# debbiemarkslab/BEAR

Measured on AMD Instinct MI355X. Metric: k-mer contexts/sec (DM-marginal+grad h), k=13, higher is better.
Workload: dtype f64

## Files before the change

### bear_amd/csrc/kernels_plan.h

```cpp
#pragma once
#include "plan_common.h"

__global__ __launch_bounds__(256) void plan_scan_kernel(const uint32_t *__restrict__ counts, uint64_t n_rows, int ncol,
                                                        uint8_t *__restrict__ quad_light,
                                                        unsigned long long *__restrict__ heavy_counts,
                                                        unsigned long long *__restrict__ hist) {
  __shared__ uint32_t s_heavy[3];
  __shared__ uint32_t s_hist[2 * SRT_NKEY];
  __shared__ uint32_t s_big[PLN_NBIG + 1];
  __shared__ unsigned long long s_total, s_cells;
  __shared__ uint32_t s_cmax;
  unsigned long long my_total = 0ull;
  uint32_t my_cells = 0u, my_cmax = 0u;
  if (threadIdx.x == 0) {
    s_total = s_cells = 0ull;
    s_cmax = 0u;
  }
  if (threadIdx.x < 3) s_heavy[threadIdx.x] = 0;
  if (threadIdx.x < 2 * SRT_NKEY) s_hist[threadIdx.x] = 0;
  for (uint32_t k = threadIdx.x; k <= PLN_NBIG; k += 256) s_big[k] = 0;
  __syncthreads();
  const uint64_t n_quads = (n_rows + PLN_QUAD - 1) / PLN_QUAD;
  for (uint64_t g = (uint64_t)blockIdx.x * 256 + threadIdx.x; g < n_quads; g += (uint64_t)gridDim.x * 256) {
    uint32_t light = 0, qhc = 0, qhr = 0;
// ... 154 lines not shown
    }
    meta[1] = run;
    meta[2] = run > 0xffffffffull ? 1ull : 0ull;
  }
  __syncthreads();
  unsigned long long off = part[threadIdx.x];
  for (uint64_t t = lo; t < hi; ++t) {
    tiles[t].off16 = (uint32_t)off;
    off += tiles[t].blk16;
  }
}

__global__ __launch_bounds__(1024) void plan_fill_kernel(const uint32_t *__restrict__ counts, uint64_t n_rows, int ncol,
                                                         const pln_tile *__restrict__ tiles, uint64_t n_tiles,
                                                         unsigned char *__restrict__ stream,
                                                         pln_heavy_col *__restrict__ heavy_col,
                                                         pln_heavy_row *__restrict__ heavy_row,
                                                         uint64_t *__restrict__ heavy_stop,
                                                         unsigned long long *__restrict__ cursors) {
  constexpr int RPT = (PLN_RMAX + 1023) / 1024;
  __shared__ uint32_t hist[SRT_NHIST];
  __shared__ uint32_t offs[SRT_NHIST];
  __shared__ uint32_t scan[16];
  __shared__ uint16_t sorted[PLN_NI + 64];
  __shared__ uint32_t s_hc, s_hr;
#ifdef BEAR_DET_BUILD
  __shared__ uint32_t comp[PLN_NI];
  static_assert((PLN_NI & (PLN_NI - 1)) == 0 && PLN_NI <= 2048, "bitonic sort over the tile's items: PLN_NI / 2 pairs, at most one per thread");
  __shared__ unsigned long long hkey[PLN_HCAP], htmp[PLN_HCAP];
#endif
  const uint32_t tid = threadIdx.x, rep = tid & (SRT_REP - 1);
  for (uint64_t t = blockIdx.x; t < n_tiles; t += gridDim.x) {
    const pln_tile ti = tiles[t];
    const uint32_t rows = ti.rows_items >> 16, n_light = ti.rows_items & 0xffffu;
    const uint32_t hc_cap = ti.hc_hr >> 16, hr_cap = ti.hc_hr & 0xffffu;
    const pln_layout L = pln_block_layout(rows, n_light, hc_cap, hr_cap);
    unsigned char *blk = stream + (size_t)ti.off16 * 16;
    uint16_t *E = reinterpret_cast<uint16_t *>(blk);
    uint8_t *nrow = blk + L.nrow;
    uint16_t *items = reinterpret_cast<uint16_t *>(blk + L.items);
    uint16_t *hoff = reinterpret_cast<uint16_t *>(blk + L.hoff);
    uint32_t *hcnt = reinterpret_cast<uint32_t *>(blk + L.hcnt);
    uint16_t *hrow = reinterpret_cast<uint16_t *>(blk + L.hrow);
    double *hn = reinterpret_cast<double *>(blk + L.hn);
    if (tid < SRT_NHIST) hist[tid] = 0;
    if (tid == 0) {
      s_hc = 0;
      s_hr = 0;
    }
    __syncthreads();
#ifdef BEAR_DET_BUILD
    uint32_t det_hc[RPT], det_hr[RPT];
    {
      uint32_t base_c = 0, base_r = 0;
#pragma unroll
      for (int k = 0; k < RPT; ++k) {
        const uint32_t lr = tid + 1024u * k;
        uint32_t nc = 0, nr = 0;
        if (lr < rows) {
          double n = 0.0;
          for (int b = 0; b < 5; ++b) {
            const uint32_t cv = counts[(ti.row0 + lr) * 5 + b];
            n += (double)cv;
            nc += (b < ncol && cv > SRT_CL) ? 1u : 0u;
          }
          nr = n > (double)SRT_CL ? 1u : 0u;
        }
        const uint32_t packed = nc | (nr << 16);
        const int lane = tid & 63, wave = tid >> 6;
        uint32_t incl = packed;
#pragma unroll
        for (int off = 1; off < 64; off <<= 1) {
          const uint32_t o = (uint32_t)__shfl_up((int)incl, off, 64);
          if (lane >= off) incl += o;
        }
        __syncthreads();
        if (lane == 63) scan[wave] = incl;
        __syncthreads();
        uint32_t before = 0, total = 0;
        for (int w = 0; w < 16; ++w) {
          if (w < wave) before += scan[w];
          total += scan[w];
        }
        const uint32_t excl = before + incl - packed;
        det_hc[k] = base_c + (excl & 0xffffu);
        det_hr[k] = base_r + (excl >> 16);
        base_c += total & 0xffffu;
        base_r += total >> 16;
      }
      __syncthreads();
      if (tid == 0) {
        s_hc = base_c;
        s_hr = base_r;
      }
    }
#endif
    uint32_t c[RPT][5], rank[RPT][5];
#pragma unroll
    for (int k = 0; k < RPT; ++k) {
      const uint32_t lr = tid + 1024u * k;
#pragma unroll
      for (int b = 0; b < 5; ++b) {
        c[k][b] = 0;
        rank[k][b] = 0;
      }
      if (lr < rows) {
        const uint64_t r = ti.row0 + lr;
        double n = 0.0;
#pragma unroll
        for (int b = 0; b < 5; ++b) {
          c[k][b] = counts[r * 5 + b];
          n += (double)c[k][b];
        }
        nrow[lr] = n < 1.0 ? (uint8_t)0 : (n <= (double)SRT_CL ? (uint8_t)n : (uint8_t)255);
        if (n > (double)SRT_CL) {
#ifdef BEAR_DET_BUILD
          const uint32_t k2 = hr_cap ? det_hr[k] : 0xffffffffu;
#else
          const uint32_t k2 = hr_cap ? atomicAdd(&s_hr, 1u) : 0xffffffffu;
#endif
          if (k2 < hr_cap) {
            hrow[k2] = (uint16_t)lr;
            hn[k2] = n;
          } else {
            const unsigned long long q = atomicAdd(&cursors[1], 1ull);
            heavy_row[q].row = r;
            heavy_row[q].n = n;
          }
        }
        if (ncol == 4 && c[k][4] > SRT_CL) heavy_stop[atomicAdd(&cursors[2], 1ull)] = c[k][4];
#pragma unroll
        for (int b = 0; b < 5; ++b) {
          if (b >= ncol) c[k][b] = 0;
          if (c[k][b] > SRT_CL) {
#ifdef BEAR_DET_BUILD
            const uint32_t k2 = hc_cap ? det_hc[k]++ : 0xffffffffu;
#else
            const uint32_t k2 = hc_cap ? atomicAdd(&s_hc, 1u) : 0xffffffffu;
#endif
            if (k2 < hc_cap) {
              hoff[k2] = (uint16_t)(lr * 5 + b);
              hcnt[k2] = c[k][b];
            } else {
              const unsigned long long q = atomicAdd(&cursors[0], 1ull);
              heavy_col[q].off = r * 5 + b;
              heavy_col[q].c = c[k][b];
            }
            c[k][b] = 0;
          }
          if (c[k][b] != 0) rank[k][b] = atomicAdd(&hist[(c[k][b] - 1) * SRT_REP + rep], 1u);
        }
      } else if (lr < ((rows + 15u) & ~15u)) {
        nrow[lr] = 0;
      }
    }
    __syncthreads();
    {
      const uint32_t v = tid < SRT_NHIST ? hist[tid] : 0u;
      const int lane = tid & 63, wave = tid >> 6;
      uint32_t incl = v;
#pragma unroll
      for (int off = 1; off < 64; off <<= 1) {
        uint32_t o = (uint32_t)__shfl_up((int)incl, off, 64);
        if (lane >= off) incl += o;
      }
      if (lane == 63) scan[wave] = incl;
      __syncthreads();
      uint32_t base = 0;
      for (int w = 0; w < wave; ++w) base += scan[w];
      if (tid < SRT_NHIST) offs[tid] = base + incl - v;
    }
    __syncthreads();
    if (tid < 30) E[tid] = (uint16_t)(tid < SRT_CL ? offs[tid * SRT_REP] : n_light);
    if (tid == 30) E[30] = (uint16_t)hc_cap;
    if (tid == 31) E[31] = (uint16_t)hr_cap;
#pragma unroll
    for (int k = 0; k < RPT; ++k)
#pragma unroll
      for (int b = 0; b < 5; ++b)
        if (c[k][b] != 0) sorted[offs[(c[k][b] - 1) * SRT_REP + rep] + rank[k][b]] = (uint16_t)((tid + 1024u * k) * 5 + b);
    __syncthreads();
#ifdef BEAR_DET_BUILD
    {
      for (uint32_t i = tid; i < PLN_NI; i += 1024) {
        uint32_t key = 0;
        for (uint32_t q = 1; q < SRT_CL; ++q) key += offs[q * SRT_REP] <= i ? 1u : 0u;
        comp[i] = i < n_light ? (key << 16) | sorted[i] : 0xffffffffu;
      }
      __syncthreads();
      for (uint32_t size = 2; size <= PLN_NI; size <<= 1)
        for (uint32_t stride = size >> 1; stride > 0; stride >>= 1) {
          const uint32_t lo = 2u * tid - (tid & (stride - 1u)), hi = lo + stride;
          if (tid < PLN_NI / 2) {
            const bool up = (lo & size) == 0u;
            const uint32_t a = comp[lo], bq = comp[hi];
            if ((a > bq) == up) {
              comp[lo] = bq;
              comp[hi] = a;
            }
          }
          __syncthreads();
        }
      for (uint32_t i = tid; i < n_light; i += 1024) sorted[i] = (uint16_t)(comp[i] & 0xffffu);
      __syncthreads();
      const uint32_t nhc = s_hc < hc_cap ? s_hc : hc_cap, nhr = s_hr < hr_cap ? s_hr : hr_cap;
      if (tid < nhc) hkey[tid] = ((unsigned long long)hoff[tid] << 32) | hcnt[tid];
      __syncthreads();
      if (tid < nhc) {
        uint32_t r = 0;
        for (uint32_t q = 0; q < nhc; ++q) r += hkey[q] < hkey[tid] ? 1u : 0u;
        htmp[r] = hkey[tid];
      }
      __syncthreads();
      if (tid < nhc) {
        hoff[tid] = (uint16_t)(htmp[tid] >> 32);
        hcnt[tid] = (uint32_t)htmp[tid];
      }
      __syncthreads();
      if (tid < nhr) hkey[tid] = ((unsigned long long)hrow[tid] << 48) | tid;
      if (tid < nhr) htmp[tid] = (unsigned long long)__double_as_longlong(hn[tid]);
      __syncthreads();
      uint32_t r = 0;
      unsigned long long mine = 0ull, myn = 0ull;
      if (tid < nhr) {
        for (uint32_t q = 0; q < nhr; ++q) r += hkey[q] < hkey[tid] ? 1u : 0u;
        mine = hkey[tid];
        myn = htmp[tid];
      }
      __syncthreads();
      if (tid < nhr) {
        hrow[r] = (uint16_t)(mine >> 48);
        hn[r] = __longlong_as_double((long long)myn);
      }
      __syncthreads();
    }
#endif
    const uint32_t padded = (n_light + 63u) & ~63u;
    for (uint32_t i = tid; i < padded; i += 1024) items[i] = i < n_light ? sorted[i] : (uint16_t)PLN_SENTINEL;
    __syncthreads();
  }
}

__global__ __launch_bounds__(1024) void plan_live_kernel(const pln_tile *__restrict__ tiles, uint64_t n_tiles,
                                                         const unsigned char *__restrict__ stream, uint16_t *__restrict__ live) {
  constexpr int RPT = (PLN_RMAX + 1023) / 1024;
  __shared__ uint32_t cnt[RPT * 16];
  const uint32_t tid = threadIdx.x, lane = tid & 63, wave = tid >> 6;
  for (uint64_t t = blockIdx.x; t < n_tiles; t += gridDim.x) {
    const pln_tile ti = tiles[t];
    const uint32_t rows = ti.rows_items >> 16;
    const uint8_t *nrow = stream + (size_t)ti.off16 * 16 + 64;
    uint16_t *out = live + t * PLN_LIVE_STRIDE;
    unsigned long long mask[RPT];
#pragma unroll
    for (int k = 0; k < RPT; ++k) {
      const uint32_t lr = tid + 1024u * k;
      mask[k] = __builtin_amdgcn_ballot_w64(lr < rows && nrow[lr] != 0);
      if (lane == 0) cnt[k * 16 + wave] = (uint32_t)__builtin_popcountll(mask[k]);
    }
    __syncthreads();
    uint32_t total = 0;
#pragma unroll
    for (int k = 0; k < RPT; ++k) {
      uint32_t base = total;
      for (int w = 0; w < 16; ++w) {
        const uint32_t c = cnt[k * 16 + w];
        if (w < (int)wave) base += c;
        total += c;
      }
      if ((mask[k] >> lane) & 1ull) out[1 + base + (uint32_t)__builtin_popcountll(mask[k] & ((1ull << lane) - 1ull))] = (uint16_t)(tid + 1024u * k);
    }
    if (tid == 0) out[0] = (uint16_t)total;
    __syncthreads();
  }
}

template <bool NORM, bool AR>
__global__ __launch_bounds__(PLN_THREADS, 4) void dm_prior_plan_kernel(const double *__restrict__ prior,
                                                                                    uint64_t n_rows, bear_params prm_arg,
                                                                                    pln_view pv,
                                                                                    const double2 *__restrict__ logtab_g,
                                                                                    double *__restrict__ partials,
                                                                                    const bear_step_io io
#ifdef PLN_STAMPS
                                                                                    , unsigned long long *__restrict__ dbg
#endif
                                                                                    ) {
  extern __shared__ __attribute__((aligned(16))) unsigned char srt_smem[];
  pln_lds_n &S = *reinterpret_cast<pln_lds_n *>(srt_smem);
  const bear_params prm = bear_params_of(prm_arg, io);
  const uint32_t tid = threadIdx.x, lane = tid & 63, wave = srt_uniform(tid >> 6);
  const double u = prm.inv_h, eps = prm.eps, eps5 = 5.0 * prm.eps;
  double acc[2] = {0.0, 0.0};

  if (tid < BEAR_LOGTAB_N) S.logtab[tid] = logtab_g[tid];
  if (tid < SRT_NKEY) {
    const bear_dp o = srt_general_fast(u + eps5, (double)(tid + 1), logtab_g);
    S.tabD[tid] = o.D;
    S.tabP[tid] = o.P;
  }
  if (tid < PLN_NBUF) {
    S.buf[tid].pri[PLN_SENTINEL] = 1.0;
    S.ticket[tid] = PLN_TICKET_START(PLN_WAVES - PLN_DMA_WAVES);
    S.sum_fail[tid] = 0xffffffffu;
  }

  const bool dma_wave = wave >= PLN_WAVES - PLN_DMA_WAVES;
  const uint32_t dw = wave - (PLN_WAVES - PLN_DMA_WAVES);
  constexpr bool GEN = !NORM && !AR;
  constexpr bool NT = GEN && PLN_GEN_NT;
  auto stage = [&](const pln_tile &ti, uint32_t b, bool with_nrow) {
    const uint32_t rows = ti.rows_items >> 16;
    if (rows == 0) return;
    const uint32_t pbytes = (rows * 40u) & ~15u, bbytes = ti.blk16 * 16u;
    const unsigned char *psrc = reinterpret_cast<const unsigned char *>(prior + ti.row0 * 5);
    const unsigned char *bsrc = pv.stream + (size_t)ti.off16 * 16;
    if (GEN && dw == 0 && lane == 0) S.nrow_in[b] = with_nrow ? 1u : 0u;
    if (!GEN || with_nrow) {
      for (uint32_t pc = dw; (pc << 10) < bbytes; pc += PLN_DMA_WAVES) pln_dma_piece<NT>(S.buf[b].blk, bsrc, bbytes, pc, lane);
    } else {
      const uint32_t items0 = pln_block_layout(rows, ti.rows_items & 0xffffu, ti.hc_hr >> 16, ti.hc_hr & 0xffffu).items;
      if (dw == PLN_DMA_WAVES - 1) pln_dma_piece<NT>(S.buf[b].blk, bsrc, 64u, 0u, lane);
      for (uint32_t pc = dw; (pc << 10) < bbytes - items0; pc += PLN_DMA_WAVES)
        pln_dma_piece<NT>(S.buf[b].blk + items0, bsrc + items0, bbytes - items0, pc, lane);
    }
    for (uint32_t pc = dw; (pc << 10) < pbytes; pc += PLN_DMA_WAVES) pln_dma_piece<NT>(S.buf[b].pri, psrc, pbytes, pc, lane);
    if (dw == 0 && ((rows * 40u) & 15u)) {
      const __attribute__((address_space(4))) double *tail =
          (const __attribute__((address_space(4))) double *)(uintptr_t)(prior + (ti.row0 + rows) * 5 - 1);
      const double v = *tail;
      if (lane == 0) S.buf[b].pri[rows * 5 - 1] = v;
    }
  };

  constexpr uint32_t PF_INSTR = (NORM || AR || PLN_GEN_PREFETCH) ? PLN_PREFETCH_KIB / 8u : 0u;
  auto prefetch_behind = [&](const pln_tile &ti) -> uint32_t {
    const uint32_t rows = ti.rows_items >> 16;
    if (PF_INSTR == 0 || rows == 0) return 0u;
    const uint64_t end_bytes = n_rows * 40ull, base = (ti.row0 + rows) * 40ull;
    const uint32_t m = srt_uniform((uint32_t)(uintptr_t)S.pf_scratch);
    uint32_t issued = 0;
    for (uint32_t k = dw; k < PF_INSTR; k += PLN_DMA_WAVES) {
      uint64_t off = base + ((uint64_t)(k * 64u + lane) << 7);
      if (off + 4u > end_bytes) off = end_bytes - 4u;
      const unsigned char *g = reinterpret_cast<const unsigned char *>(prior) + off;
      uint32_t keep_m0;
      asm volatile("s_mov_b32 %0, m0\n\ts_mov_b32 m0, %2\n\ts_nop 0\n\tglobal_load_lds_dword %1, off\n\ts_mov_b32 m0, %0"
                   : "=&s"(keep_m0)
                   : "v"(g), "s"(m)
                   : "memory");
      ++issued;
    }
    return issued;
  };
  uint32_t pf_young = 0;
#ifdef PLN_STAMPS
  unsigned long long tph[8] = {0, 0, 0, 0, 0, 0, 0, 0}, t_prev = __builtin_amdgcn_s_memtime();
  int prev_kind = 0;
#define PLN_STAMP(k)                                              \
  {                                                               \
    const unsigned long long now = __builtin_amdgcn_s_memtime();  \
    tph[k] += now - t_prev;                                       \
    t_prev = now;                                                 \
  }
#else
#define PLN_STAMP(k)
#endif
  static_assert(PLN_NBUF == 2, "the DMA-wave protocol below is written for a two-slot ring");
  const uint64_t G = gridDim.x;
  const uint64_t first = (pv.n_tiles * (uint64_t)blockIdx.x) / G, count = (pv.n_tiles * ((uint64_t)blockIdx.x + 1)) / G - first;
  auto fetch_desc = [&](uint64_t j0) {
    if (dw == 0 && j0 < count)
      pln_dma_piece(S.desc[(j0 >> 5) & 1u], pv.tiles + first + j0, PLN_DESC_CHUNK * (uint32_t)sizeof(pln_tile), 0u, lane);
  };
  if (dma_wave) {
    __builtin_amdgcn_s_setprio(3);
    fetch_desc(0);
    fetch_desc(PLN_DESC_CHUNK);
    srt_wait_dma();
  }
  __syncthreads();
  pln_tile cur = pln_desc(S.desc, 0, count), nxt = pln_desc(S.desc, 1, count);
  if (dma_wave) stage(cur, 0, !PLN_GEN_NROW_ON_DEMAND);
  uint32_t slot = 0;
  for (uint64_t j = 0; j < count; ++j) {
#ifdef PLN_STAMPS
    PLN_STAMP(prev_kind)
    prev_kind = 4;
#endif
    if (dma_wave) pln_wait_all_but(pf_young);
    PLN_STAMP(1)
    srt_sync();
    PLN_STAMP(2)
    const pln_tile nn = pln_desc(S.desc, j + 2, count);
    if (dma_wave) {
      if ((j & (PLN_DESC_CHUNK - 1)) == 0 && j != 0) fetch_desc(j + PLN_DESC_CHUNK);
      stage(nxt, slot ^ 1u, !GEN || !PLN_GEN_NROW_ON_DEMAND || srt_uniform(S.sum_fail[slot ^ 1u]) == (uint32_t)j);
      pf_young = prefetch_behind(nxt);
      cur = nxt;
      nxt = nn;
      slot ^= 1u;
      continue;
    }
    PLN_STAMP(3)

    const pln_buf_n &B = S.buf[slot];
    const uint32_t rows = cur.rows_items >> 16, n_light = cur.rows_items & 0xffffu;
    const uint32_t hc = cur.hc_hr >> 16, hr = cur.hc_hr & 0xffffu;
    const pln_layout L = pln_block_layout(rows, n_light, hc, hr);
    const uint16_t *E = reinterpret_cast<const uint16_t *>(B.blk);
    const uint8_t *nrow = B.blk + L.nrow;
    const uint16_t *items = reinterpret_cast<const uint16_t *>(B.blk + L.items);
    if (tid == 0) S.ticket[(slot + 1) % PLN_NBUF] = PLN_TICKET_START(PLN_WAVES - PLN_DMA_WAVES);
    const uint32_t n_hcu = (hc + 63u) >> 6, n_hru = AR ? 0u : (hr + 63u) >> 6, n_heavy = n_hcu + n_hru;
    const uint32_t n_units = (n_light + 63u) >> 6;
    const uint32_t n_work = n_heavy + n_units;
    static_assert(PLN_CHUNK == 128, "two adjacent contexts per lane");
    for (uint32_t c = wave; GEN && c * PLN_CHUNK < rows; c += PLN_WAVES - PLN_DMA_WAVES) {
      const uint32_t row0c = c * PLN_CHUNK + 2u * lane;
      const uint32_t rr = row0c < rows ? row0c : 0u;
      const double2 *src = reinterpret_cast<const double2 *>(&B.pri[rr * 5]);
      const double2 v0 = src[0], v1 = src[1], v2 = src[2], v3 = src[3], v4 = src[4];
      const double S5[2] = {((v0.x + v0.y) + (v1.x + v1.y)) + v2.x, ((v2.y + v3.x) + (v3.y + v4.x)) + v4.y};
      bool bad[2];
#pragma unroll
      for (int q = 0; q < 2; ++q) bad[q] = row0c + q < rows && !(__builtin_fabs(S5[q] - 1.0) <= SRT_SUM1_TOL);
      if (__builtin_amdgcn_ballot_w64(bad[0] || bad[1])) {
        if (lane == 0) S.sum_fail[slot] = (uint32_t)(j + 1);
        uint32_t nn_[2];
        if (!PLN_GEN_NROW_ON_DEMAND || srt_uniform(S.nrow_in[slot])) {
#pragma unroll
          for (int q = 0; q < 2; ++q) nn_[q] = bad[q] ? (uint32_t)nrow[rr + q] : 0u;
        } else {
          const uint8_t *g = pv.stream + (size_t)cur.off16 * 16 + L.nrow;
#pragma unroll
          for (int q = 0; q < 2; ++q) nn_[q] = bad[q] ? (uint32_t)g[rr + q] : 0u;
        }
#pragma unroll
        for (int q = 0; q < PLN_CHUNK / 64; ++q) {
          const uint32_t own = nn_[q] == 255u ? 0u : nn_[q];
          if (__builtin_amdgcn_ballot_w64(own != 0)) {
            uint32_t cm = own;
#pragma unroll
            for (int off = 32; off > 0; off >>= 1) {
              const uint32_t o2 = (uint32_t)__shfl_xor((int)cm, off, 64);
              cm = o2 > cm ? o2 : cm;
            }
            const double xa[1] = {own ? __builtin_fma(S5[q], u, eps5) : 1.0};
            const uint32_t ca[1] = {own};
            bear_dp o[1];
            srt_light<1>(xa, ca, 0u, srt_uniform(cm), S.logtab, o);
            if (own) {
              acc[0] += S.tabD[own - 1] - o[0].D;
              acc[1] = __builtin_fma(xa[0] - eps5, o[0].P, __builtin_fma(-u, S.tabP[own - 1], acc[1]));
            }
          }
        }
      }
    }
    PLN_FOR_UNITS_F(w, &S.ticket[slot], n_work, wave, PLN_WAVES - PLN_DMA_WAVES) {
#ifdef PLN_STAMPS
      {
        const unsigned long long now = __builtin_amdgcn_s_memtime();
        tph[prev_kind] += now - t_prev;
        t_prev = now;
        prev_kind = w < n_heavy ? 5 : 6;
      }
#endif
      if (w < n_hcu) {
        const uint32_t i = w * 64u + lane;
        if (i < hc) {
          const uint32_t off = reinterpret_cast<const uint16_t *>(B.blk + L.hoff)[i];
          const double cnt = (double)reinterpret_cast<const uint32_t *>(B.blk + L.hcnt)[i];
          if (AR) {
            acc[0] = __builtin_fma(cnt, bear_log_tab(B.pri[off] + eps, S.logtab), acc[0]);
          } else {
            const double x = __builtin_fma(B.pri[off], u, eps);
            const bear_dp o = srt_general_fast(x, cnt, S.logtab);
            acc[0] += o.D;
            acc[1] = __builtin_fma(eps - x, o.P, acc[1]);
          }
        }
        continue;
      }
      if (w < n_heavy) {
        const uint32_t i = (w - n_hcu) * 64u + lane;
        if (i < hr) {
          const double *f = &B.pri[(uint32_t)reinterpret_cast<const uint16_t *>(B.blk + L.hrow)[i] * 5u];
          const double A = NORM ? u + eps5 : __builtin_fma(((f[0] + f[1]) + (f[2] + f[3])) + f[4], u, eps5);
          const bear_dp o = srt_general_fast(A, reinterpret_cast<const double *>(B.blk + L.hn)[i], S.logtab);
          acc[0] -= o.D;
          acc[1] = __builtin_fma(A - eps5, o.P, acc[1]);
        }
        continue;
      }
      {
        const uint32_t un = n_heavy + n_units - 1u - w;
        uint32_t cmin, cmax;
        const uint32_t ci[1] = {pln_unit_counts(E, n_light, un, lane, &cmin, &cmax)};
        const uint32_t off = items[un * 64u + lane];
        if (AR) {
          acc[0] = __builtin_fma((double)ci[0], bear_log_tab(B.pri[off] + eps, S.logtab), acc[0]);
          continue;
        }
        const double x[1] = {__builtin_fma(B.pri[off], u, eps)};
        bear_dp o[1];
        srt_light<1>(x, ci, cmin, cmax, S.logtab, o);
        acc[0] += o[0].D;
        acc[1] = __builtin_fma(eps - x[0], o[0].P, acc[1]);
        continue;
      }
    }
    cur = nxt;
    nxt = nn;
    slot ^= 1u;
  }
  srt_wait_dma();
#ifdef PLN_STAMPS
  if (lane == 0 && dbg) {
    for (int k = 0; k < 8; ++k) dbg[((size_t)blockIdx.x * PLN_WAVES + wave) * 8 + k] = tph[k];
  }
#endif
  const uint64_t gtid = (uint64_t)blockIdx.x * PLN_THREADS + tid, gsz = (uint64_t)gridDim.x * PLN_THREADS;
  for (uint64_t i = gtid; i < pv.n_heavy_col; i += gsz) {
    const pln_heavy_col h = pv.heavy_col[i];
    if (AR) {
      acc[0] = __builtin_fma((double)h.c, bear_log_tab(prior[h.off] + eps, S.logtab), acc[0]);
      continue;
    }
    const double x = __builtin_fma(prior[h.off], u, eps);
    const bear_dp o = srt_general_fast(x, (double)h.c, S.logtab);
    acc[0] += o.D;
    acc[1] = __builtin_fma(eps - x, o.P, acc[1]);
  }
  for (uint64_t i = gtid; !AR && i < pv.n_heavy_row; i += gsz) {
    const pln_heavy_row h = pv.heavy_row[i];
    const double *f = prior + h.row * 5;
    const double A = __builtin_fma(((f[0] + f[1]) + (f[2] + f[3])) + f[4], u, eps5);
    const bear_dp o = srt_general_fast(A, h.n, S.logtab);
    acc[0] -= o.D;
    acc[1] = __builtin_fma(A - eps5, o.P, acc[1]);
  }
  if (!AR && blockIdx.x == 0 && tid < SRT_CL) {
    const double m = (double)pv.hist[tid];
    acc[0] -= m * S.tabD[tid];
    acc[1] = __builtin_fma(u * m, S.tabP[tid], acc[1]);
  }
  __syncthreads();
  block_finish<2>(acc, partials, io);
}

struct pln_buf_r {
  uint32_t ref[PLN_RMAX * 5 + 4];
  __attribute__((aligned(16))) unsigned char blk[PLN_BLOCK_MAX];
};
#define PLN_RSLOT 3
struct pln_lds_r {
  pln_buf_r buf[PLN_RSLOT];
  double2 logtab[BEAR_LOGTAB_N];
  double tabD[2][SRT_NKEY];
  double tabP[2][SRT_NKEY];
  uint32_t meta[PLN_RSLOT][2];
  uint32_t ticket[PLN_RSLOT];
  uint32_t landed[PLN_RSLOT];
  uint32_t left[PLN_RSLOT];
};

template <bool AR>
__global__ __launch_bounds__(PLN_THREADS, 4) void dm_ref_plan_kernel(const uint32_t *__restrict__ ref,
                                                                                  uint64_t n_rows, bear_params prm_arg,
                                                                                  pln_view pv,
                                                                                  const double2 *__restrict__ logtab_g,
                                                                                  double *__restrict__ partials,
                                                                                  const bear_step_io io, const bear_apply_io apply) {
  extern __shared__ __attribute__((aligned(16))) unsigned char srt_smem[];
  pln_lds_r &S = *reinterpret_cast<pln_lds_r *>(srt_smem);
  const bear_params prm = bear_params_of(prm_arg, io);
  const uint32_t tid = threadIdx.x, lane = tid & 63, wave = srt_uniform(tid >> 6);
  const double u = prm.inv_h, eps = prm.eps;
  const double A = u + 5.0 * eps;
  const double x4 = prm.nw * prm.V * u + eps;
  const double VU = prm.V * u;
  const double tau = prm.tau;
  const double w2c = tau * (eps + 0.25 * VU);
  const double nwV = prm.nw * prm.V;
  double acc[4] = {0.0, 0.0, 0.0, 0.0};

  if (tid < BEAR_LOGTAB_N) S.logtab[tid] = logtab_g[tid];
  if (tid < 2 * SRT_NKEY) {
    const int which = tid / SRT_NKEY, j = tid % SRT_NKEY;
    const bear_dp o = srt_general_fast(which ? x4 : A, (double)(j + 1), logtab_g);
    S.tabD[which][j] = o.D;
    S.tabP[which][j] = o.P;
  }
  if (tid < PLN_RSLOT) {
    S.landed[tid] = S.left[tid] = 0u;
    S.ticket[tid] = PLN_TICKET_START(PLN_WAVES - PLN_DMA_WAVES);
  }
  if (tid < 4 * PLN_RSLOT) S.buf[tid >> 2].ref[PLN_SENTINEL + (tid & 3)] = 0;

  const bool dma_wave = wave >= PLN_WAVES - PLN_DMA_WAVES;
  const uint32_t dw = wave - (PLN_WAVES - PLN_DMA_WAVES);
  constexpr uint32_t CWAVES = PLN_WAVES - PLN_DMA_WAVES;
  auto stage = [&](const pln_tile &ti, uint32_t b) {
    const uint32_t rows = ti.rows_items >> 16;
    const uint32_t rbytes = rows * 20u, rb16 = rbytes & ~15u, bbytes = ti.blk16 * 16u;
    const unsigned char *rsrc = reinterpret_cast<const unsigned char *>(ref + ti.row0 * 5);
    const unsigned char *bsrc = pv.stream + (size_t)ti.off16 * 16;
    for (uint32_t pc = 0; (pc << 10) < bbytes; ++pc) pln_dma_piece(S.buf[b].blk, bsrc, bbytes, pc, lane);
    for (uint32_t pc = 0; (pc << 10) < rb16; ++pc) pln_dma_piece(S.buf[b].ref, rsrc, rb16, pc, lane);
    if (rbytes & 15u) {
      const uint32_t w0 = rb16 >> 2, nw = (rbytes & 15u) >> 2;
      const __attribute__((address_space(4))) uint32_t *tail =
          (const __attribute__((address_space(4))) uint32_t *)(uintptr_t)(ref + ti.row0 * 5 + w0);
      const uint32_t v0 = tail[0], v1 = nw > 1 ? tail[1] : 0u, v2 = nw > 2 ? tail[2] : 0u;
      if (lane == 0) {
        S.buf[b].ref[w0] = v0;
        if (nw > 1) S.buf[b].ref[w0 + 1] = v1;
        if (nw > 2) S.buf[b].ref[w0 + 2] = v2;
      }
    }
    if (lane == 0) {
      S.meta[b][0] = ti.rows_items;
      S.meta[b][1] = ti.hc_hr;
      S.ticket[b] = PLN_TICKET_START(PLN_WAVES - PLN_DMA_WAVES);
    }
  };
  auto alpha_from = [&](double rb, double R) {
    const double dev = __builtin_fma(rb + eps, bear_rcp(R), -0.25);
    return __builtin_fma(__builtin_fma(prm.E, dev, 0.25), VU, eps);
  };
  auto accumulate = [&](double x, const bear_dp &o) {
    const double w1 = eps - x;
    acc[0] += o.D;
    acc[1] = __builtin_fma(w1, o.P, acc[1]);
    acc[2] = __builtin_fma(__builtin_fma(-tau, x, w2c), o.P, acc[2]);
    acc[3] = __builtin_fma(nwV * w1, o.P, acc[3]);
  };
  auto accumulate_ar = [&](double rb, double R, double c) {
    const double dev = __builtin_fma(rb + eps, bear_rcp(R), -0.25);
    const double f = __builtin_fma(prm.E, dev, 0.25) * prm.V;
    const double p = f + eps;
    const double dLdf = c * bear_rcp(p);
    acc[0] = __builtin_fma(c, bear_log_tab(p, S.logtab), acc[0]);
    acc[2] = __builtin_fma(dLdf, -prm.tauE * dev * prm.V, acc[2]);
    acc[3] = __builtin_fma(dLdf, -nwV * f, acc[3]);
  };

  const uint64_t G = gridDim.x;
  const uint64_t first = (pv.n_tiles * (uint64_t)blockIdx.x) / G, count = (pv.n_tiles * ((uint64_t)blockIdx.x + 1)) / G - first;
  __syncthreads();
  if (dma_wave) {
    __builtin_amdgcn_s_setprio(3);
    pln_tile ti = pln_load_tile(pv, dw < count ? first + dw : pv.n_tiles);
    for (uint64_t j = dw; j < count; j += PLN_DMA_WAVES) {
      const uint32_t b = (uint32_t)(j % PLN_RSLOT), gen = (uint32_t)(j / PLN_RSLOT);
      const pln_tile ti_next = pln_load_tile(pv, j + PLN_DMA_WAVES < count ? first + j + PLN_DMA_WAVES : pv.n_tiles);
      while (pln_peek(&S.left[b]) < CWAVES * gen) __builtin_amdgcn_s_sleep(1);
      stage(ti, b);
      srt_wait_dma();
      asm volatile("s_waitcnt lgkmcnt(0)" ::: "memory");
      if (lane == 0) atomicAdd(&S.landed[b], 1u);
      ti = ti_next;
    }
  }
  for (uint64_t j = 0; !dma_wave && j < count; ++j) {
    const uint32_t slot = (uint32_t)(j % PLN_RSLOT), gen = (uint32_t)(j / PLN_RSLOT);
    while (pln_peek(&S.landed[slot]) < gen + 1u) __builtin_amdgcn_s_sleep(1);
    const pln_buf_r &B = S.buf[slot];
    const uint32_t rows_items = srt_uniform(S.meta[slot][0]), hc_hr = srt_uniform(S.meta[slot][1]);
    const uint32_t rows = rows_items >> 16, n_light = rows_items & 0xffffu;
    const uint32_t hc = hc_hr >> 16;
    const pln_layout L = pln_block_layout(rows, n_light, hc, hc_hr & 0xffffu);
    const uint16_t *E = reinterpret_cast<const uint16_t *>(B.blk);
    const uint16_t *items = reinterpret_cast<const uint16_t *>(B.blk + L.items);
    const uint32_t n_hcu = (hc + 63u) >> 6;
    const uint32_t n_units = (n_light + 63u) >> 6;
    PLN_FOR_UNITS_F(w, &S.ticket[slot], n_hcu + n_units, wave, CWAVES) {
      if (w < n_hcu) {
        const uint32_t i = w * 64u + lane;
        if (i < hc) {
          const uint32_t off = reinterpret_cast<const uint16_t *>(B.blk + L.hoff)[i];
          const uint32_t *rr = &B.ref[((off * 52429u) >> 18) * 5u];
          const double R = (double)(((uint64_t)rr[0] + rr[1]) + ((uint64_t)rr[2] + rr[3])) + 4.0 * eps;
          const double cnt = (double)reinterpret_cast<const uint32_t *>(B.blk + L.hcnt)[i];
          if (AR) {
            accumulate_ar((double)B.ref[off], R, cnt);
          } else {
            const double x = alpha_from((double)B.ref[off], R);
            accumulate(x, srt_general_fast(x, cnt, S.logtab));
          }
        }
        continue;
      }
      const uint32_t un = n_hcu + n_units - 1u - w;
      uint32_t cmin, cmax;
      const uint32_t ci[1] = {pln_unit_counts(E, n_light, un, lane, &cmin, &cmax)};
      const uint32_t off = items[un * 64u + lane];
      const uint32_t *rr = &B.ref[((off * 52429u) >> 18) * 5u];
      const double R = (double)(((uint64_t)rr[0] + rr[1]) + ((uint64_t)rr[2] + rr[3])) + 4.0 * eps;
      if (AR) {
        accumulate_ar((double)B.ref[off], R, (double)ci[0]);
        continue;
      }
      const double x[1] = {alpha_from((double)B.ref[off], R)};
      bear_dp o[1];
      srt_light<1>(x, ci, cmin, cmax, S.logtab, o);
      accumulate(x[0], o[0]);
    }
    asm volatile("s_waitcnt lgkmcnt(0)" ::: "memory");
    if (lane == 0) atomicAdd(&S.left[slot], 1u);
  }
  srt_wait_dma();
  const uint64_t gtid = (uint64_t)blockIdx.x * PLN_THREADS + tid, gsz = (uint64_t)gridDim.x * PLN_THREADS;
  for (uint64_t i = gtid; i < pv.n_heavy_col; i += gsz) {
    const pln_heavy_col h = pv.heavy_col[i];
    const uint32_t *rr = ref + (h.off / 5) * 5;
    const double R = (double)(((uint64_t)rr[0] + rr[1]) + ((uint64_t)rr[2] + rr[3])) + 4.0 * eps;
    if (AR) {
      accumulate_ar((double)ref[h.off], R, (double)h.c);
      continue;
    }
    const double x = alpha_from((double)ref[h.off], R);
    accumulate(x, srt_general_fast(x, (double)h.c, S.logtab));
  }
  if (AR) {
    const double f4 = nwV, p4 = f4 + eps;
    double c4sum = 0.0;
    if (blockIdx.x == 0 && tid < SRT_CL) c4sum = (double)(tid + 1) * (double)pv.hist[SRT_NKEY + tid];
    for (uint64_t i = gtid; i < pv.n_heavy_stop; i += gsz) c4sum += (double)pv.heavy_stop[i];
    acc[0] = __builtin_fma(c4sum, bear_log_tab(p4, S.logtab), acc[0]);
    acc[3] = __builtin_fma(c4sum * bear_rcp(p4), nwV * (1.0 - f4), acc[3]);
    __syncthreads();
    block_finish<4>(acc, partials, io, apply);
    return;
  }
  for (uint64_t i = gtid; i < pv.n_heavy_row; i += gsz) {
    const double n = pv.heavy_row[i].n;
    if (pln_in_big_hist(pv, n)) continue;
    const bear_dp o = srt_general_fast(A, n, S.logtab);
    acc[0] -= o.D;
    acc[1] = __builtin_fma(u, o.P, acc[1]);
  }
  pln_big_totals(pv, A, u, gtid, gsz, S.logtab, acc[0], acc[1]);
  for (uint64_t i = gtid; i < pv.n_heavy_stop; i += gsz) {
    const bear_dp o = srt_general_fast(x4, (double)pv.heavy_stop[i], S.logtab);
    acc[0] += o.D;
    acc[1] = __builtin_fma(eps - x4, o.P, acc[1]);
    acc[3] = __builtin_fma(VU * nwV, o.P, acc[3]);
  }
  if (blockIdx.x == 0 && tid < SRT_CL) {
    const double mn = (double)pv.hist[tid], m4 = (double)pv.hist[SRT_NKEY + tid];
    acc[0] -= mn * S.tabD[0][tid];
    acc[1] = __builtin_fma(u * mn, S.tabP[0][tid], acc[1]);
    const double P4 = m4 * S.tabP[1][tid];
    acc[0] += m4 * S.tabD[1][tid];
    acc[1] = __builtin_fma(eps - x4, P4, acc[1]);
    acc[3] = __builtin_fma(VU * nwV, P4, acc[3]);
  }
  __syncthreads();
  block_finish<4>(acc, partials, io, apply);
}

struct pln_lds_g {
  double pri[PLN_RMAX * 5 + 2];
  double grad[PLN_RMAX * 5 + 2];
  __attribute__((aligned(16))) unsigned char blk[PLN_BLOCK_MAX];
  double2 logtab[BEAR_LOGTAB_N];
  double tabD[SRT_NKEY];
  double tabP[SRT_NKEY];
  uint32_t ticket;
  __attribute__((aligned(16))) uint32_t pf_scratch[64];
};
static_assert(sizeof(pln_lds_g) <= 158 * 1024, "gradient-row kernel: LDS budget");

__device__ __forceinline__ void pln_touch_lines(uint32_t *scratch, const void *src, uint32_t bytes, uint32_t k, uint32_t lane) {
  const uint32_t off = (k * 64u + lane) << 7;
  if (off < bytes) {
    const unsigned char *g = static_cast<const unsigned char *>(src) + off;
    const uint32_t m = srt_uniform((uint32_t)(uintptr_t)scratch);
    uint32_t keep_m0;
    asm volatile("s_mov_b32 %0, m0\n\ts_mov_b32 m0, %2\n\ts_nop 0\n\tglobal_load_lds_dword %1, off\n\ts_mov_b32 m0, %0"
                 : "=&s"(keep_m0)
                 : "v"(g), "s"(m)
                 : "memory");
  }
}

template <bool NORM, bool AR>
__global__ __launch_bounds__(PLN_THREADS, 4) void dm_prior_plan_grad_kernel(const double *__restrict__ prior,
                                                                                         bear_params prm_arg, pln_view pv,
                                                                                         const double2 *__restrict__ logtab_g,
                                                                                         double *__restrict__ grad_out,
                                                                                         double *__restrict__ partials,
                                                                                         const bear_step_io io) {
  extern __shared__ __attribute__((aligned(16))) unsigned char srt_smem[];
  pln_lds_g &S = *reinterpret_cast<pln_lds_g *>(srt_smem);
  const bear_params prm = bear_params_of(prm_arg, io);
  const uint32_t tid = threadIdx.x, lane = tid & 63, wave = srt_uniform(tid >> 6);
  const double u = prm.inv_h, eps = prm.eps, eps5 = 5.0 * prm.eps;
  double acc[2] = {0.0, 0.0};
  if (tid < BEAR_LOGTAB_N) S.logtab[tid] = logtab_g[tid];
  if (tid < SRT_NKEY) {
    const bear_dp o = srt_general_fast(u + eps5, (double)(tid + 1), logtab_g);
    S.tabD[tid] = o.D;
    S.tabP[tid] = o.P;
  }
  if (tid == 0) {
    S.pri[PLN_SENTINEL] = 1.0;
    S.ticket = PLN_TICKET_START(PLN_WAVES);
  }
  pln_tile nxt = pln_load_tile(pv, blockIdx.x);
  for (uint64_t t = blockIdx.x; t < pv.n_tiles; t += gridDim.x) {
    const pln_tile cur = nxt;
    const uint32_t rows = cur.rows_items >> 16, n_light = cur.rows_items & 0xffffu;
    const uint32_t hc = cur.hc_hr >> 16, hr = cur.hc_hr & 0xffffu;
    const pln_layout L = pln_block_layout(rows, n_light, hc, hr);
    __syncthreads();
    {
// ... 311 lines not shown
```

### bear_amd/csrc/plan_common.h

```cpp
#pragma once
#include "sorted_common.h"

#ifndef PLN_THREADS
#define PLN_THREADS 1024
#endif
#define PLN_WAVES (PLN_THREADS / 64)
#ifndef PLN_UNITS
#define PLN_UNITS 32
#endif
#define PLN_NI (PLN_UNITS * 64)
#ifndef PLN_NI_CUT
#define PLN_NI_CUT PLN_NI
#endif
#ifndef PLN_RMAX
#define PLN_RMAX 1664
#endif
#ifndef PLN_HCAP
#define PLN_HCAP 128
#endif
#define PLN_NBIG 4096
#define PLN_BLOCKS_PER_CU (1024 / PLN_THREADS)
#define PLN_QUAD 4
#define PLN_LIVE_STRIDE (PLN_RMAX + 8)
#define PLN_SENTINEL (PLN_RMAX * 5)
#ifndef PLN_NBUF
#define PLN_NBUF 2
#endif
#define PLN_BLOCK_MAX (64 + PLN_RMAX + PLN_NI * 2 + PLN_HCAP * (2 + 4 + 2 + 8))

struct pln_tile {
  uint64_t row0;
  uint32_t rows_items;
  uint32_t off16;
  uint32_t hc_hr;
  uint32_t blk16;
  uint64_t pad;
};
static_assert(sizeof(pln_tile) == 32, "tile descriptors are fetched with one s_load_dwordx8");
#ifndef PLN_CHUNK
#define PLN_CHUNK 128
#endif
#ifndef PLN_DMA_WAVES
#define PLN_DMA_WAVES 2
#endif
#ifndef PLN_PREFETCH_KIB
#define PLN_PREFETCH_KIB 24
#endif
#ifndef PLN_GEN_PREFETCH
#define PLN_GEN_PREFETCH 1
#endif
#ifndef PLN_GEN_NT
#define PLN_GEN_NT 0
#endif
#ifndef PLN_GEN_NROW_ON_DEMAND
#define PLN_GEN_NROW_ON_DEMAND 1
#endif
#define PLN_DESC_CHUNK 32
#define PLN_DESC_PAD (2 * PLN_DESC_CHUNK)

struct pln_layout {
  uint32_t nrow, items, hoff, hcnt, hrow, hn, end;
};
__host__ __device__ inline pln_layout pln_block_layout(uint32_t rows, uint32_t n_light, uint32_t hc, uint32_t hr) {
  pln_layout L;
  L.nrow = 64u;
  L.items = L.nrow + ((rows + 15u) & ~15u);
  L.hoff = L.items + (((n_light + 63u) & ~63u) * 2u);
  L.hcnt = L.hoff + (((hc + 7u) & ~7u) * 2u);
  L.hrow = L.hcnt + (((hc + 3u) & ~3u) * 4u);
  L.hn = L.hrow + (((hr + 7u) & ~7u) * 2u);
  L.end = L.hn + (((hr + 1u) & ~1u) * 8u);
  return L;
}

struct pln_heavy_col {
  uint64_t off;
  uint64_t c;
};

struct pln_heavy_row {
  uint64_t row;
  double n;
};

struct pln_view {
  const pln_tile *tiles;
  const unsigned char *stream;
  const pln_heavy_col *heavy_col;
  const pln_heavy_row *heavy_row;
  const uint64_t *heavy_stop;
  const unsigned long long *hist;
  const unsigned long long *hist_big;
  int big_in_hist;
  uint64_t n_tiles, n_heavy_col, n_heavy_row, n_heavy_stop;
  const uint16_t *live;
  const uint16_t *live2;
  int subset;
};

__device__ __forceinline__ void pln_big_totals(const pln_view &pv, double A, double scale, uint64_t gtid, uint64_t gsz, const double2 *logtab,
                                               double &acc_D, double &acc_P) {
  if (!pv.hist_big) return;
  for (uint64_t n = SRT_CL + 1 + gtid; n <= PLN_NBIG; n += gsz) {
    const unsigned long long m = pv.hist_big[n];
    if (m) {
      const bear_dp o = srt_general_fast(A, (double)n, logtab);
      acc_D -= (double)m * o.D;
      acc_P = __builtin_fma(scale * (double)m, o.P, acc_P);
    }
  }
}
__device__ __forceinline__ bool pln_in_big_hist(const pln_view &pv, double n) { return pv.big_in_hist && n <= (double)PLN_NBIG; }

__device__ __forceinline__ uint32_t pln_dma(void *lds, const void *src, uint32_t bytes, uint32_t wave, uint32_t lane,
                                            uint32_t first) {
  const uint32_t d = (uint32_t)(uintptr_t)lds;
  const unsigned char *s = static_cast<const unsigned char *>(src) + lane * 16u;
  const uint32_t pieces = (bytes + 1023u) >> 10;
  uint32_t issued = 0;
  for (uint32_t piece = (wave + PLN_WAVES - (first % PLN_WAVES)) % PLN_WAVES; piece < pieces; piece += PLN_WAVES) {
    const unsigned char *g = s + (piece << 10);
    const uint32_t m = srt_uniform(d + (piece << 10));
    if ((piece << 10) + lane * 16u < bytes)
      {
      uint32_t keep_m0;
      asm volatile("s_mov_b32 %0, m0\n\ts_mov_b32 m0, %2\n\ts_nop 0\n\tglobal_load_lds_dwordx4 %1, off\n\ts_mov_b32 m0, %0"
                   : "=&s"(keep_m0)
                   : "v"(g), "s"(m)
                   : "memory");
    }
    ++issued;
  }
  return issued;
}

template <bool NT = false>
__device__ __forceinline__ void pln_dma_piece(void *lds, const void *src, uint32_t bytes, uint32_t piece, uint32_t lane) {
  const uint32_t m = srt_uniform((uint32_t)(uintptr_t)lds + (piece << 10));
  const unsigned char *g = static_cast<const unsigned char *>(src) + (piece << 10) + lane * 16u;
  if ((piece << 10) + lane * 16u < bytes)
    {
      uint32_t keep_m0;
      if (NT)
        asm volatile("s_mov_b32 %0, m0\n\ts_mov_b32 m0, %2\n\ts_nop 0\n\tglobal_load_lds_dwordx4 %1, off nt\n\ts_mov_b32 m0, %0"
                     : "=&s"(keep_m0)
                     : "v"(g), "s"(m)
                     : "memory");
      else
        asm volatile("s_mov_b32 %0, m0\n\ts_mov_b32 m0, %2\n\ts_nop 0\n\tglobal_load_lds_dwordx4 %1, off\n\ts_mov_b32 m0, %0"
                     : "=&s"(keep_m0)
                     : "v"(g), "s"(m)
                     : "memory");
    }
}

__device__ __forceinline__ void pln_wait_all_but(uint32_t younger) {
  switch (younger) {
    case 0: asm volatile("s_waitcnt vmcnt(0)" ::: "memory"); break;
    case 1: asm volatile("s_waitcnt vmcnt(1)" ::: "memory"); break;
    case 2: asm volatile("s_waitcnt vmcnt(2)" ::: "memory"); break;
    case 3: asm volatile("s_waitcnt vmcnt(3)" ::: "memory"); break;
    case 4: asm volatile("s_waitcnt vmcnt(4)" ::: "memory"); break;
    case 5: asm volatile("s_waitcnt vmcnt(5)" ::: "memory"); break;
    case 6: asm volatile("s_waitcnt vmcnt(6)" ::: "memory"); break;
    case 7: asm volatile("s_waitcnt vmcnt(7)" ::: "memory"); break;
    case 8: asm volatile("s_waitcnt vmcnt(8)" ::: "memory"); break;
    default: asm volatile("s_waitcnt vmcnt(0)" ::: "memory"); break;
  }
}

__device__ __forceinline__ pln_tile pln_load_tile(const pln_view &pv, uint64_t t) {
  pln_tile ti;
  ti.row0 = 0;
  ti.rows_items = 0;
  ti.off16 = 0;
  ti.hc_hr = 0;
  ti.blk16 = 0;
  ti.pad = 0;
  if (t < pv.n_tiles) {
    const __attribute__((address_space(4))) pln_tile *tc = (const __attribute__((address_space(4))) pln_tile *)(uintptr_t)pv.tiles;
    ti.row0 = tc[t].row0;
    ti.rows_items = tc[t].rows_items;
    ti.off16 = tc[t].off16;
    ti.hc_hr = tc[t].hc_hr;
    ti.blk16 = tc[t].blk16;
    ti.pad = tc[t].pad;
  }
  return ti;
}

__device__ __forceinline__ uint32_t pln_ticket(uint32_t *counter, uint32_t lane) {
  uint32_t t = 0;
  if (lane == 0)
    asm volatile("ds_add_rtn_u32 %0, %1, %2\n\ts_waitcnt lgkmcnt(0)" : "=&v"(t) : "v"((uint32_t)(uintptr_t)counter), "v"(1u) : "memory");
  return srt_uniform(t);
}

#ifdef BEAR_DET_BUILD
#define PLN_FOR_UNITS(w, counter, n, first, stride) for (uint32_t w = (first); w < (n); w += (stride))
#else
#define PLN_FOR_UNITS(w, counter, n, first, stride) for (uint32_t w = pln_ticket(counter, lane); w < (n); w = pln_ticket(counter, lane))
#endif
#if defined(BEAR_DET_BUILD) || defined(PLN_NO_FIRST_UNIT_DEALT)
#define PLN_FOR_UNITS_F(w, counter, n, first, stride) PLN_FOR_UNITS(w, counter, n, first, stride)
#define PLN_TICKET_START(stride) 0u
#else
#define PLN_FOR_UNITS_F(w, counter, n, first, stride) for (uint32_t w = (first); w < (n); w = pln_ticket(counter, lane))
#define PLN_TICKET_START(stride) ((uint32_t)(stride))
#endif

__device__ __forceinline__ uint32_t pln_ticket_issue(uint32_t *counter, uint32_t lane) {
  uint32_t t = 0;
  if (lane == 0) t = atomicAdd(counter, 1u);
  return t;
}

__device__ __forceinline__ uint32_t pln_unit_counts(const uint16_t *E, uint32_t n_light, uint32_t un, uint32_t lane,
                                                    uint32_t *cmin, uint32_t *cmax) {
  const uint32_t base = un * 64u, idx = base + lane;
  const uint32_t last = (base + 64u <= n_light ? base + 64u : n_light) - 1u;
  const uint32_t e = lane < 30u ? (uint32_t)E[lane] : 0xffffffffu;
  uint32_t lo, hi;
  asm("s_bcnt1_i32_b64 %0, %1" : "=s"(lo) : "s"(__builtin_amdgcn_ballot_w64(e <= base)) : "scc");
  asm("s_bcnt1_i32_b64 %0, %1" : "=s"(hi) : "s"(__builtin_amdgcn_ballot_w64(e <= last)) : "scc");
  uint32_t c = lo;
  for (uint32_t k = lo; k < hi; ++k) c += idx >= (uint32_t)__builtin_amdgcn_readlane((int)e, (int)k) ? 1u : 0u;
  *cmin = base + 64u <= n_light ? lo : 0u;
  *cmax = hi;
  return idx < n_light ? c : 0u;
}

struct pln_buf_n {
  double pri[PLN_RMAX * 5 + 2];
  __attribute__((aligned(16))) unsigned char blk[PLN_BLOCK_MAX];
};
struct pln_lds_n {
  pln_buf_n buf[PLN_NBUF];
  double2 logtab[BEAR_LOGTAB_N];
  double tabD[SRT_NKEY];
  double tabP[SRT_NKEY];
  uint32_t ticket[PLN_NBUF];
  uint32_t sum_fail[PLN_NBUF];
  uint32_t nrow_in[PLN_NBUF];
  __attribute__((aligned(16))) pln_tile desc[2][PLN_DESC_CHUNK];
  __attribute__((aligned(16))) uint32_t pf_scratch[64];
};
static_assert(sizeof(pln_lds_n) <= 160 * 1024, "one block per CU: the planned mode-N kernels' LDS");

__device__ __forceinline__ pln_tile pln_desc(const pln_tile (*ring)[PLN_DESC_CHUNK], uint64_t j, uint64_t count) {
  pln_tile ti;
  ti.row0 = 0;
  ti.rows_items = 0;
  ti.off16 = 0;
  ti.hc_hr = 0;
  ti.blk16 = 0;
  ti.pad = 0;
  if (j < count) {
    const uint32_t *d = reinterpret_cast<const uint32_t *>(&ring[(j >> 5) & 1u][j & 31u]);
    const uint32_t lo = srt_uniform(d[0]), hi = srt_uniform(d[1]);
    ti.row0 = ((uint64_t)hi << 32) | lo;
    ti.rows_items = srt_uniform(d[2]);
    ti.off16 = srt_uniform(d[3]);
    ti.hc_hr = srt_uniform(d[4]);
    ti.blk16 = srt_uniform(d[5]);
  }
  return ti;
}

__device__ __forceinline__ uint32_t pln_peek(const uint32_t *p) {
  return srt_uniform(__hip_atomic_load(p, __ATOMIC_RELAXED, __HIP_MEMORY_SCOPE_WORKGROUP));
}
```

Baseline: 136.9 billion.

## Replace block-wide barrier ring with per-slot flag producer/consumer flow between DMA and compute waves

Under a new default-on PLN_FLOW mode, each of the two DMA waves owns one ring slot and stages every other tile. Compute waves spin on per-slot LDS 'landed' counters instead of a block-wide __syncthreads per tile, and signal completion through 'left' counters. Tile metadata is passed through LDS, so the descriptor-chunk DMA ring goes away. The intent is to decouple producer and consumer waves, removing the per-tile barrier stall. In exchange it adds spin-waiting with s_sleep and reduces staging parallelism per tile to a single wave.

```diff
diff --git a/bear_amd/csrc/kernels_plan.h b/bear_amd/csrc/kernels_plan.h
--- a/bear_amd/csrc/kernels_plan.h
+++ b/bear_amd/csrc/kernels_plan.h
@@ -480,30 +480,39 @@
   if (tid < PLN_NBUF) {
     S.buf[tid].pri[PLN_SENTINEL] = 1.0;
     S.ticket[tid] = PLN_TICKET_START(PLN_WAVES - PLN_DMA_WAVES);
+#if PLN_FLOW
+    S.sum_fail[tid] = 0u;
+    S.landed[tid] = S.left[tid] = 0u;
+#else
     S.sum_fail[tid] = 0xffffffffu;
+#endif
   }
 
   const bool dma_wave = wave >= PLN_WAVES - PLN_DMA_WAVES;
   const uint32_t dw = wave - (PLN_WAVES - PLN_DMA_WAVES);
   constexpr bool GEN = !NORM && !AR;
   constexpr bool NT = GEN && PLN_GEN_NT;
+  constexpr uint32_t DSTEP = PLN_FLOW ? 1u : (uint32_t)PLN_DMA_WAVES;
+  const uint32_t d0 = PLN_FLOW ? 0u : dw;
   auto stage = [&](const pln_tile &ti, uint32_t b, bool with_nrow) {
     const uint32_t rows = ti.rows_items >> 16;
     if (rows == 0) return;
     const uint32_t pbytes = (rows * 40u) & ~15u, bbytes = ti.blk16 * 16u;
     const unsigned char *psrc = reinterpret_cast<const unsigned char *>(prior + ti.row0 * 5);
     const unsigned char *bsrc = pv.stream + (size_t)ti.off16 * 16;
+#if !PLN_FLOW
     if (GEN && dw == 0 && lane == 0) S.nrow_in[b] = with_nrow ? 1u : 0u;
+#endif
     if (!GEN || with_nrow) {
-      for (uint32_t pc = dw; (pc << 10) < bbytes; pc += PLN_DMA_WAVES) pln_dma_piece<NT>(S.buf[b].blk, bsrc, bbytes, pc, lane);
+      for (uint32_t pc = d0; (pc << 10) < bbytes; pc += DSTEP) pln_dma_piece<NT>(S.buf[b].blk, bsrc, bbytes, pc, lane);
     } else {
       const uint32_t items0 = pln_block_layout(rows, ti.rows_items & 0xffffu, ti.hc_hr >> 16, ti.hc_hr & 0xffffu).items;
-      if (dw == PLN_DMA_WAVES - 1) pln_dma_piece<NT>(S.buf[b].blk, bsrc, 64u, 0u, lane);
-      for (uint32_t pc = dw; (pc << 10) < bbytes - items0; pc += PLN_DMA_WAVES)
+      if (PLN_FLOW || dw == PLN_DMA_WAVES - 1) pln_dma_piece<NT>(S.buf[b].blk, bsrc, 64u, 0u, lane);
+      for (uint32_t pc = d0; (pc << 10) < bbytes - items0; pc += DSTEP)
         pln_dma_piece<NT>(S.buf[b].blk + items0, bsrc + items0, bbytes - items0, pc, lane);
     }
-    for (uint32_t pc = dw; (pc << 10) < pbytes; pc += PLN_DMA_WAVES) pln_dma_piece<NT>(S.buf[b].pri, psrc, pbytes, pc, lane);
-    if (dw == 0 && ((rows * 40u) & 15u)) {
+    for (uint32_t pc = d0; (pc << 10) < pbytes; pc += DSTEP) pln_dma_piece<NT>(S.buf[b].pri, psrc, pbytes, pc, lane);
+    if ((PLN_FLOW || dw == 0) && ((rows * 40u) & 15u)) {
       const __attribute__((address_space(4))) double *tail =
           (const __attribute__((address_space(4))) double *)(uintptr_t)(prior + (ti.row0 + rows) * 5 - 1);
       const double v = *tail;
@@ -512,13 +521,12 @@
   };
 
   constexpr uint32_t PF_INSTR = (NORM || AR || PLN_GEN_PREFETCH) ? PLN_PREFETCH_KIB / 8u : 0u;
-  auto prefetch_behind = [&](const pln_tile &ti) -> uint32_t {
-    const uint32_t rows = ti.rows_items >> 16;
+  auto prefetch_from = [&](uint64_t row, uint32_t rows) -> uint32_t {
     if (PF_INSTR == 0 || rows == 0) return 0u;
-    const uint64_t end_bytes = n_rows * 40ull, base = (ti.row0 + rows) * 40ull;
+    const uint64_t end_bytes = n_rows * 40ull, base = row * 40ull;
     const uint32_t m = srt_uniform((uint32_t)(uintptr_t)S.pf_scratch);
     uint32_t issued = 0;
-    for (uint32_t k = dw; k < PF_INSTR; k += PLN_DMA_WAVES) {
+    for (uint32_t k = d0; k < PF_INSTR; k += DSTEP) {
       uint64_t off = base + ((uint64_t)(k * 64u + lane) << 7);
       if (off + 4u > end_bytes) off = end_bytes - 4u;
       const unsigned char *g = reinterpret_cast<const unsigned char *>(prior) + off;
@@ -544,9 +552,52 @@
 #else
 #define PLN_STAMP(k)
 #endif
-  static_assert(PLN_NBUF == 2, "the DMA-wave protocol below is written for a two-slot ring");
+  static_assert(PLN_NBUF == 2 && PLN_DMA_WAVES == 2, "the DMA-wave protocols below are written for a two-slot ring and two DMA waves");
   const uint64_t G = gridDim.x;
   const uint64_t first = (pv.n_tiles * (uint64_t)blockIdx.x) / G, count = (pv.n_tiles * ((uint64_t)blockIdx.x + 1)) / G - first;
+#if PLN_FLOW
+  constexpr uint32_t CWAVES = PLN_WAVES - PLN_DMA_WAVES;
+  __syncthreads();
+  if (dma_wave) {
+    __builtin_amdgcn_s_setprio(3);
+    pln_tile ti = pln_load_tile(pv, dw < count ? first + dw : pv.n_tiles);
+    for (uint64_t j = dw; j < count; j += PLN_DMA_WAVES) {
+      const uint32_t gen = (uint32_t)(j / PLN_NBUF);
+      const pln_tile ti_next = pln_load_tile(pv, j + PLN_DMA_WAVES < count ? first + j + PLN_DMA_WAVES : pv.n_tiles);
+      PLN_STAMP(0)
+      while (pln_peek(&S.left[dw]) < CWAVES * gen) __builtin_amdgcn_s_sleep(1);
+      PLN_STAMP(2)
+      const bool with_nrow = !GEN || !PLN_GEN_NROW_ON_DEMAND || srt_uniform(S.sum_fail[dw]) != 0u;
+      stage(ti, dw, with_nrow);
+      pf_young = prefetch_from(ti_next.row0, ti_next.rows_items >> 16);
+      if (lane == 0) {
+        S.meta[dw][0] = ti.rows_items;
+        S.meta[dw][1] = ti.hc_hr;
+        S.meta[dw][2] = ti.off16;
+        S.meta[dw][3] = with_nrow ? 1u : 0u;
+        S.ticket[dw] = PLN_TICKET_START(PLN_WAVES - PLN_DMA_WAVES);
+        S.sum_fail[dw] = 0u;
+      }
+      PLN_STAMP(3)
+      pln_wait_all_but(pf_young);
+      asm volatile("s_waitcnt lgkmcnt(0)" ::: "memory");
+      if (lane == 0) atomicAdd(&S.landed[dw], 1u);
+      PLN_STAMP(1)
+      ti = ti_next;
+    }
+  }
+  for (uint64_t j = 0; !dma_wave && j < count; ++j) {
+    const uint32_t slot = (uint32_t)(j % PLN_NBUF), gen = (uint32_t)(j / PLN_NBUF);
+#ifdef PLN_STAMPS
+    PLN_STAMP(prev_kind)
+    prev_kind = 4;
+#endif
+    while (pln_peek(&S.landed[slot]) < gen + 1u) __builtin_amdgcn_s_sleep(1);
+    PLN_STAMP(2)
+    const uint32_t t_rows_items = srt_uniform(S.meta[slot][0]), t_hc_hr = srt_uniform(S.meta[slot][1]);
+#define PLN_TILE_OFF16 srt_uniform(S.meta[slot][2])
+#define PLN_TILE_NROW_IN srt_uniform(S.meta[slot][3])
+#else
   auto fetch_desc = [&](uint64_t j0) {
     if (dw == 0 && j0 < count)
       pln_dma_piece(S.desc[(j0 >> 5) & 1u], pv.tiles + first + j0, PLN_DESC_CHUNK * (uint32_t)sizeof(pln_tile), 0u, lane);
@@ -574,22 +625,26 @@
     if (dma_wave) {
       if ((j & (PLN_DESC_CHUNK - 1)) == 0 && j != 0) fetch_desc(j + PLN_DESC_CHUNK);
       stage(nxt, slot ^ 1u, !GEN || !PLN_GEN_NROW_ON_DEMAND || srt_uniform(S.sum_fail[slot ^ 1u]) == (uint32_t)j);
-      pf_young = prefetch_behind(nxt);
+      pf_young = prefetch_from(nxt.row0 + (nxt.rows_items >> 16), nxt.rows_items >> 16);
       cur = nxt;
       nxt = nn;
       slot ^= 1u;
       continue;
     }
     PLN_STAMP(3)
+    const uint32_t t_rows_items = cur.rows_items, t_hc_hr = cur.hc_hr;
+#define PLN_TILE_OFF16 cur.off16
+#define PLN_TILE_NROW_IN srt_uniform(S.nrow_in[slot])
+    if (tid == 0) S.ticket[(slot + 1) % PLN_NBUF] = PLN_TICKET_START(PLN_WAVES - PLN_DMA_WAVES);
+#endif
 
     const pln_buf_n &B = S.buf[slot];
-    const uint32_t rows = cur.rows_items >> 16, n_light = cur.rows_items & 0xffffu;
-    const uint32_t hc = cur.hc_hr >> 16, hr = cur.hc_hr & 0xffffu;
+    const uint32_t rows = t_rows_items >> 16, n_light = t_rows_items & 0xffffu;
+    const uint32_t hc = t_hc_hr >> 16, hr = t_hc_hr & 0xffffu;
     const pln_layout L = pln_block_layout(rows, n_light, hc, hr);
     const uint16_t *E = reinterpret_cast<const uint16_t *>(B.blk);
     const uint8_t *nrow = B.blk + L.nrow;
     const uint16_t *items = reinterpret_cast<const uint16_t *>(B.blk + L.items);
-    if (tid == 0) S.ticket[(slot + 1) % PLN_NBUF] = PLN_TICKET_START(PLN_WAVES - PLN_DMA_WAVES);
     const uint32_t n_hcu = (hc + 63u) >> 6, n_hru = AR ? 0u : (hr + 63u) >> 6, n_heavy = n_hcu + n_hru;
     const uint32_t n_units = (n_light + 63u) >> 6;
     const uint32_t n_work = n_heavy + n_units;
@@ -604,13 +659,13 @@
 #pragma unroll
       for (int q = 0; q < 2; ++q) bad[q] = row0c + q < rows && !(__builtin_fabs(S5[q] - 1.0) <= SRT_SUM1_TOL);
       if (__builtin_amdgcn_ballot_w64(bad[0] || bad[1])) {
-        if (lane == 0) S.sum_fail[slot] = (uint32_t)(j + 1);
+        if (lane == 0) S.sum_fail[slot] = PLN_FLOW ? 1u : (uint32_t)(j + 1);
         uint32_t nn_[2];
-        if (!PLN_GEN_NROW_ON_DEMAND || srt_uniform(S.nrow_in[slot])) {
+        if (!PLN_GEN_NROW_ON_DEMAND || PLN_TILE_NROW_IN) {
 #pragma unroll
           for (int q = 0; q < 2; ++q) nn_[q] = bad[q] ? (uint32_t)nrow[rr + q] : 0u;
         } else {
-          const uint8_t *g = pv.stream + (size_t)cur.off16 * 16 + L.nrow;
+          const uint8_t *g = pv.stream + (size_t)PLN_TILE_OFF16 * 16 + L.nrow;
 #pragma unroll
           for (int q = 0; q < 2; ++q) nn_[q] = bad[q] ? (uint32_t)g[rr + q] : 0u;
         }
@@ -689,10 +744,17 @@
         continue;
       }
     }
+#if PLN_FLOW
+    asm volatile("s_waitcnt lgkmcnt(0)" ::: "memory");
+    if (lane == 0) atomicAdd(&S.left[slot], 1u);
+#else
     cur = nxt;
     nxt = nn;
     slot ^= 1u;
-  }
+#endif
+  }
+#undef PLN_TILE_OFF16
+#undef PLN_TILE_NROW_IN
   srt_wait_dma();
 #ifdef PLN_STAMPS
   if (lane == 0 && dbg) {
diff --git a/bear_amd/csrc/plan_common.h b/bear_amd/csrc/plan_common.h
--- a/bear_amd/csrc/plan_common.h
+++ b/bear_amd/csrc/plan_common.h
@@ -54,6 +54,9 @@
 #endif
 #ifndef PLN_GEN_NROW_ON_DEMAND
 #define PLN_GEN_NROW_ON_DEMAND 1
+#endif
+#ifndef PLN_FLOW
+#define PLN_FLOW 1
 #endif
 #define PLN_DESC_CHUNK 32
 #define PLN_DESC_PAD (2 * PLN_DESC_CHUNK)
@@ -241,8 +244,14 @@
   double tabP[SRT_NKEY];
   uint32_t ticket[PLN_NBUF];
   uint32_t sum_fail[PLN_NBUF];
+#if PLN_FLOW
+  uint32_t landed[PLN_NBUF];
+  uint32_t left[PLN_NBUF];
+  uint32_t meta[PLN_NBUF][4];
+#else
   uint32_t nrow_in[PLN_NBUF];
   __attribute__((aligned(16))) pln_tile desc[2][PLN_DESC_CHUNK];
+#endif
   __attribute__((aligned(16))) uint32_t pf_scratch[64];
 };
 static_assert(sizeof(pln_lds_n) <= 160 * 1024, "one block per CU: the planned mode-N kernels' LDS");
```

Measured after the change: 124.5 billion. 9.1% lower.
